# facebookresearch/esm

Hardware: NVIDIA H100
Metric: sequences/sec ESM-2 650M L=1024 embedding extract (higher is better)
Workload: dtype f16 operands, f32 accumulate/residual/LayerNorm/softmax

## Files before the change

esm_b200/csrc/attention_wg.cuh:

```cuda
#pragma once

#include "attention_common.cuh"

namespace esmb200 {

namespace attn_wg_cfg {
constexpr int BLOCK_Q = 128;
constexpr int BLOCK_KV = 128;
constexpr int STAGES = 4;
constexpr int Q_BUFS = 2;
constexpr int TILE_BYTES = 128 * 128;
constexpr int NUM_THREADS = 384;
constexpr int SMEM_BYTES = (Q_BUFS + 2 * STAGES) * TILE_BYTES + 1024 + 256;
}

__global__ void __launch_bounds__(attn_wg_cfg::NUM_THREADS, 1)
attention_wg_kernel(const __grid_constant__ CUtensorMap tmap_q, const __grid_constant__ CUtensorMap tmap_kv,
                    const AttnParams p) {
  using namespace attn_wg_cfg;
  constexpr float LOG2E = attn_cfg::LOG2E;
  constexpr int D = attn_cfg::HEAD_DIM;
  extern __shared__ uint8_t smem_raw[];
  uint8_t* smem = reinterpret_cast<uint8_t*>((reinterpret_cast<uintptr_t>(smem_raw) + 1023) & ~uintptr_t(1023));
  uint8_t* smem_q = smem;
  uint8_t* smem_k = smem + Q_BUFS * TILE_BYTES;
  uint8_t* smem_v = smem_k + STAGES * TILE_BYTES;
  uint64_t* bars = reinterpret_cast<uint64_t*>(smem_v + STAGES * TILE_BYTES);
  uint64_t* q_full = bars;
  uint64_t* q_empty = bars + Q_BUFS;
  uint64_t* k_full = bars + 2 * Q_BUFS;
  uint64_t* v_full = k_full + STAGES;
  uint64_t* kv_empty = v_full + STAGES;

  const uint32_t wg = __shfl_sync(0xffffffffu, threadIdx.x / 128, 0);
  const int nqt = (p.T + BLOCK_Q - 1) / BLOCK_Q;
  const int items = p.B * p.H * nqt;

  if (threadIdx.x == 0) {
    tma_prefetch_desc(&tmap_q);
    tma_prefetch_desc(&tmap_kv);
    for (int i = 0; i < Q_BUFS; ++i) {
      mbar_init(&q_full[i], 1);
      mbar_init(&q_empty[i], 2);
    }
    for (int i = 0; i < STAGES; ++i) {
      mbar_init(&k_full[i], 1);
      mbar_init(&v_full[i], 1);
      mbar_init(&kv_empty[i], 2);
    }
    fence_barrier_init();
  }
  __syncthreads();
  pdl_launch_dependents();
  pdl_wait();

  if (wg == 0) {
    setmaxnreg_dec<24>();
    if (threadIdx.x == 0) {
      auto wait_empty = [](uint64_t* bar, uint32_t parity) {
#if ESMB200_WATCHDOG
        uint32_t polls = 0;
        while (!mbar_try_wait(bar, parity)) {
          __nanosleep(64);
          if (++polls == (1u << 24)) __trap();
        }
#else
        while (!mbar_try_wait(bar, parity)) __nanosleep(64);
#endif
      };
      uint32_t qi = 0, it = 0;
      for (int w = blockIdx.x; w < items; w += gridDim.x) {
        const int qt = w % nqt, h = (w / nqt) % p.H, b = w / (nqt * p.H);
        const int nblk = (__ldg(p.kvlen + b) + BLOCK_KV - 1) / BLOCK_KV;
        if (nblk == 0) continue;
        const int row_base = (b / p.cols) * p.T;
        const int x0 = (b % p.cols) * 3 * p.E + h * D;
        const uint32_t qb = qi % Q_BUFS;
        wait_empty(&q_empty[qb], ((qi / Q_BUFS) & 1) ^ 1);
        mbar_arrive_expect_tx(&q_full[qb], TILE_BYTES);
        tma_load_2d(smem_q + qb * TILE_BYTES, &tmap_q, &q_full[qb], x0, row_base + qt * BLOCK_Q);
        ++qi;
        for (int j = 0; j < nblk; ++j, ++it) {
          const uint32_t s = it % STAGES;
          wait_empty(&kv_empty[s], ((it / STAGES) & 1) ^ 1);
          mbar_arrive_expect_tx(&k_full[s], TILE_BYTES);
          tma_load_2d(smem_k + s * TILE_BYTES, &tmap_kv, &k_full[s], x0 + p.E, row_base + j * BLOCK_KV);
          mbar_arrive_expect_tx(&v_full[s], TILE_BYTES);
          tma_load_2d(smem_v + s * TILE_BYTES, &tmap_kv, &v_full[s], x0 + 2 * p.E, row_base + j * BLOCK_KV);
        }
      }
    }
    return;
  }

  setmaxnreg_inc<240>();
  const uint32_t mw = wg - 1;
  const uint32_t warp = (threadIdx.x / 32) % 4;
  const uint32_t lane = threadIdx.x % 32, g = lane / 4, c = lane % 4;
  const bool signal = (threadIdx.x % 128) == 0;
  const uint32_t q_base = smem_u32(smem_q) + mw * 64 * 128;
  const uint32_t k_base = smem_u32(smem_k), v_base = smem_u32(smem_v);
  uint32_t qi = 0, it = 0;

  auto turn_begin = [&]() { named_bar_sync(1 + mw, 256); };
  auto turn_end = [&]() { named_bar_arrive(2 - mw, 256); };
  if (mw == 1) turn_end();

  auto wait_full = [](uint64_t* bar, uint32_t parity) {
#if ESMB200_WATCHDOG
    uint32_t polls = 0;
    while (!mbar_try_wait(bar, parity))
      if (++polls == (1u << 26)) __trap();
#else
    while (!mbar_try_wait(bar, parity)) {
    }
#endif
  };

  for (int w = blockIdx.x; w < items; w += gridDim.x) {
    const int qt = w % nqt, h = (w / nqt) % p.H, b = w / (nqt * p.H);
    const int nblk = (__ldg(p.kvlen + b) + BLOCK_KV - 1) / BLOCK_KV;
    const uint32_t* kb_ptr = p.keybits + (size_t)b * p.words;
    float o[32];
#pragma unroll
    for (int i = 0; i < 32; ++i) o[i] = 0.f;
    float m[2] = {-INFINITY, -INFINITY}, l[2] = {0.f, 0.f};

    if (nblk > 0) {
      const uint32_t qb = qi % Q_BUFS;
      const uint64_t dq = wgmma_desc_sw128(q_base + qb * TILE_BYTES);
      float sc[64];
      uint32_t pa[32];
      float alpha[2];

      auto issue_qk = [&](uint32_t s) {
        const uint64_t dk = wgmma_desc_sw128(k_base + s * TILE_BYTES);
        wgmma_fence();
#pragma unroll
        for (int k = 0; k < D / 16; ++k) wgmma_m64n128k16(sc, dq + 2 * k, dk + 2 * k, k);
        wgmma_commit();
      };
      auto issue_pv = [&](uint32_t s) {
#pragma unroll
        for (int i = 0; i < 8; ++i) {
          o[4 * i] *= alpha[0]; o[4 * i + 1] *= alpha[0];
          o[4 * i + 2] *= alpha[1]; o[4 * i + 3] *= alpha[1];
        }
        wgmma_fence();
        const uint64_t dv = wgmma_desc_sw128_mn(v_base + s * TILE_BYTES);
#pragma unroll
        for (int kk = 0; kk < BLOCK_KV / 16; ++kk) {
          const uint32_t a[4] = {pa[4 * kk], pa[4 * kk + 1], pa[4 * kk + 2], pa[4 * kk + 3]};
          wgmma_m64n64k16_rs(o, a, dv + kk * (2048 >> 4));
        }
        wgmma_commit();
      };
      auto softmax = [&](int j) {
        const uint4 kw = __ldg(reinterpret_cast<const uint4*>(kb_ptr + 4 * j));
        if ((kw.x & kw.y & kw.z & kw.w) != 0xffffffffu) {
          const uint32_t wd[4] = {kw.x, kw.y, kw.z, kw.w};
#pragma unroll
          for (int i = 0; i < 16; ++i)
#pragma unroll
            for (int e = 0; e < 2; ++e)
              if (!((wd[i / 4] >> ((i % 4) * 8 + 2 * c + e)) & 1u)) sc[4 * i + e] = sc[4 * i + 2 + e] = -INFINITY;
        }
        float mx[2][8];
#pragma unroll
        for (int i = 0; i < 8; ++i)
#pragma unroll
          for (int r = 0; r < 2; ++r)
            mx[r][i] = fmaxf(fmaxf(sc[4 * i + 2 * r], sc[4 * i + 2 * r + 1]),
                             fmaxf(sc[4 * (i + 8) + 2 * r], sc[4 * (i + 8) + 2 * r + 1]));
#pragma unroll
        for (int w = 4; w >= 1; w /= 2)
#pragma unroll
          for (int i = 0; i < w; ++i) {
            mx[0][i] = fmaxf(mx[0][i], mx[0][i + w]);
            mx[1][i] = fmaxf(mx[1][i], mx[1][i + w]);
          }
        float ref[2];
#pragma unroll
        for (int r = 0; r < 2; ++r) {
          const float mn = fmaxf(m[r], quad_max(mx[r][0]));
          alpha[r] = (mn == -INFINITY) ? 1.f : ex2_approx((m[r] - mn) * LOG2E);
          m[r] = mn;
          ref[r] = (mn == -INFINITY) ? 0.f : -mn * LOG2E;
          l[r] *= alpha[r];
        }
        float ls[2][4] = {{0.f, 0.f, 0.f, 0.f}, {0.f, 0.f, 0.f, 0.f}};
#pragma unroll
        for (int i = 0; i < 16; ++i)
#pragma unroll
          for (int r = 0; r < 2; ++r) {
            sc[4 * i + 2 * r] = ex2_approx(fmaf(sc[4 * i + 2 * r], LOG2E, ref[r]));
            sc[4 * i + 2 * r + 1] = ex2_approx(fmaf(sc[4 * i + 2 * r + 1], LOG2E, ref[r]));
            ls[r][i % 4] += sc[4 * i + 2 * r] + sc[4 * i + 2 * r + 1];
          }
#pragma unroll
        for (int r = 0; r < 2; ++r) l[r] += (ls[r][0] + ls[r][1]) + (ls[r][2] + ls[r][3]);
      };
      auto convert_p = [&]() {
#pragma unroll
        for (int i = 0; i < 16; ++i)
#pragma unroll
          for (int r = 0; r < 2; ++r) pa[2 * i + r] = pack_half2(sc[4 * i + 2 * r], sc[4 * i + 2 * r + 1]);
      };

      wait_full(&q_full[qb], (qi / Q_BUFS) & 1);
      ++qi;
      uint32_t s = it % STAGES;
      wait_full(&k_full[s], (it / STAGES) & 1);
      turn_begin();
      issue_qk(s);
      turn_end();
      wgmma_wait<0>();
      reg_fence_f(sc);
      if (nblk == 1 && signal) mbar_arrive(&q_empty[qb]);
      softmax(0);
      convert_p();
      wait_full(&v_full[s], (it / STAGES) & 1);
      for (int j = 1; j < nblk; ++j) {
        const uint32_t sp = s;
        ++it;
        s = it % STAGES;
        wait_full(&k_full[s], (it / STAGES) & 1);
        turn_begin();
        issue_qk(s);
        issue_pv(sp);
        turn_end();
        wgmma_wait<1>();
        reg_fence_f(sc);
        if (j == nblk - 1 && signal) mbar_arrive(&q_empty[qb]);
        softmax(j);
        wait_full(&v_full[s], (it / STAGES) & 1);
        wgmma_wait<0>();
        reg_fence_f(o);
        reg_fence_f(sc);
        if (signal) mbar_arrive(&kv_empty[sp]);
        convert_p();
      }
      turn_begin();
      issue_pv(s);
      turn_end();
      wgmma_wait<0>();
      reg_fence_f(o);
      if (signal) mbar_arrive(&kv_empty[s]);
      ++it;
    }

    const int row_base = (b / p.cols) * p.T;
#pragma unroll
    for (int r = 0; r < 2; ++r) {
      const float lr = quad_sum(l[r]);
      const int t = qt * BLOCK_Q + (int)(mw * 64 + warp * 16 + g + 8 * r);
      if (t >= p.T) continue;
      const float inv = lr > 0.f ? 1.0f / lr : 0.f;
      if (p.row_max != nullptr && c == 0) {
        const size_t si = ((size_t)b * p.H + h) * p.T + t;
        p.row_max[si] = m[r] == -INFINITY ? 0.f : m[r];
        p.row_sum[si] = lr;
      }
      __half* dst = p.ctx + ((size_t)(row_base + t) * p.cols + b % p.cols) * p.E + h * D;
#pragma unroll
      for (int i = 0; i < 8; ++i)
        *reinterpret_cast<__half2*>(dst + i * 8 + 2 * (int)c) =
            __floats2half2_rn(o[4 * i + 2 * r] * inv, o[4 * i + 2 * r + 1] * inv);
    }
  }
  if (mw == 0) turn_begin();
}

inline cudaError_t launch_attention_wg(const CUtensorMap& tmap_q, const CUtensorMap& tmap_kv, const AttnParams& p,
                                       int num_sms, cudaStream_t stream) {
  using namespace attn_wg_cfg;
  cudaError_t e = cudaFuncSetAttribute(attention_wg_kernel, cudaFuncAttributeMaxDynamicSharedMemorySize, SMEM_BYTES);
  if (e != cudaSuccess) return e;
  const long long items = (long long)p.B * p.H * ((p.T + BLOCK_Q - 1) / BLOCK_Q);
  if (items > 0x7fffffffLL) return cudaErrorInvalidConfiguration;
  const int grid = items < num_sms ? (int)items : num_sms;
  return launch_pdl(attention_wg_kernel, dim3(grid), dim3(NUM_THREADS), SMEM_BYTES, stream, tmap_q, tmap_kv, p);
}

}
```

Measured before the change: 320.1.

## Overlap final PV of previous tile with next tile's first QK in attention

```diff
diff --git a/esm_b200/csrc/attention_wg.cuh b/esm_b200/csrc/attention_wg.cuh
--- a/esm_b200/csrc/attention_wg.cuh
+++ b/esm_b200/csrc/attention_wg.cuh
@@ -117,148 +117,100 @@
 #endif
   };
 
-  for (int w = blockIdx.x; w < items; w += gridDim.x) {
+  float o[32];
+  float sc[64];
+  uint32_t pa[32];
+  float alpha[2];
+  float m[2] = {-INFINITY, -INFINITY}, l[2] = {0.f, 0.f};
+  float mp[2], lp[2];
+  uint64_t dq = 0;
+  const uint32_t* kb_ptr = p.keybits;
+
+  auto issue_qk = [&](uint32_t s) {
+    const uint64_t dk = wgmma_desc_sw128(k_base + s * TILE_BYTES);
+    wgmma_fence();
+#pragma unroll
+    for (int k = 0; k < D / 16; ++k) wgmma_m64n128k16(sc, dq + 2 * k, dk + 2 * k, k);
+    wgmma_commit();
+  };
+  auto issue_pv = [&](uint32_t s) {
+#pragma unroll
+    for (int i = 0; i < 8; ++i) {
+      o[4 * i] *= alpha[0]; o[4 * i + 1] *= alpha[0];
+      o[4 * i + 2] *= alpha[1]; o[4 * i + 3] *= alpha[1];
+    }
+    wgmma_fence();
+    const uint64_t dv = wgmma_desc_sw128_mn(v_base + s * TILE_BYTES);
+#pragma unroll
+    for (int kk = 0; kk < BLOCK_KV / 16; ++kk) {
+      const uint32_t a[4] = {pa[4 * kk], pa[4 * kk + 1], pa[4 * kk + 2], pa[4 * kk + 3]};
+      wgmma_m64n64k16_rs(o, a, dv + kk * (2048 >> 4));
+    }
+    wgmma_commit();
+  };
+  auto softmax = [&](int j) {
+    const uint4 kw = __ldg(reinterpret_cast<const uint4*>(kb_ptr + 4 * j));
+    if ((kw.x & kw.y & kw.z & kw.w) != 0xffffffffu) {
+      const uint32_t wd[4] = {kw.x, kw.y, kw.z, kw.w};
+#pragma unroll
+      for (int i = 0; i < 16; ++i)
+#pragma unroll
+        for (int e = 0; e < 2; ++e)
+          if (!((wd[i / 4] >> ((i % 4) * 8 + 2 * c + e)) & 1u)) sc[4 * i + e] = sc[4 * i + 2 + e] = -INFINITY;
+    }
+    float mx[2][8];
+#pragma unroll
+    for (int i = 0; i < 8; ++i)
+#pragma unroll
+      for (int r = 0; r < 2; ++r)
+        mx[r][i] = fmaxf(fmaxf(sc[4 * i + 2 * r], sc[4 * i + 2 * r + 1]),
+                         fmaxf(sc[4 * (i + 8) + 2 * r], sc[4 * (i + 8) + 2 * r + 1]));
+#pragma unroll
+    for (int w = 4; w >= 1; w /= 2)
+#pragma unroll
+      for (int i = 0; i < w; ++i) {
+        mx[0][i] = fmaxf(mx[0][i], mx[0][i + w]);
+        mx[1][i] = fmaxf(mx[1][i], mx[1][i + w]);
+      }
+    float ref[2];
+#pragma unroll
+    for (int r = 0; r < 2; ++r) {
+      const float mn = fmaxf(m[r], quad_max(mx[r][0]));
+      alpha[r] = (mn == -INFINITY) ? 1.f : ex2_approx((m[r] - mn) * LOG2E);
+      m[r] = mn;
+      ref[r] = (mn == -INFINITY) ? 0.f : -mn * LOG2E;
+      l[r] *= alpha[r];
+    }
+    float ls[2][4] = {{0.f, 0.f, 0.f, 0.f}, {0.f, 0.f, 0.f, 0.f}};
+#pragma unroll
+    for (int i = 0; i < 16; ++i)
+#pragma unroll
+      for (int r = 0; r < 2; ++r) {
+        sc[4 * i + 2 * r] = ex2_approx(fmaf(sc[4 * i + 2 * r], LOG2E, ref[r]));
+        sc[4 * i + 2 * r + 1] = ex2_approx(fmaf(sc[4 * i + 2 * r + 1], LOG2E, ref[r]));
+        ls[r][i % 4] += sc[4 * i + 2 * r] + sc[4 * i + 2 * r + 1];
+      }
+#pragma unroll
+    for (int r = 0; r < 2; ++r) l[r] += (ls[r][0] + ls[r][1]) + (ls[r][2] + ls[r][3]);
+  };
+  auto convert_p = [&]() {
+#pragma unroll
+    for (int i = 0; i < 16; ++i)
+#pragma unroll
+      for (int r = 0; r < 2; ++r) pa[2 * i + r] = pack_half2(sc[4 * i + 2 * r], sc[4 * i + 2 * r + 1]);
+  };
+  auto store = [&](int w, const float (&ls_)[2], const float (&ms_)[2]) {
     const int qt = w % nqt, h = (w / nqt) % p.H, b = w / (nqt * p.H);
-    const int nblk = (__ldg(p.kvlen + b) + BLOCK_KV - 1) / BLOCK_KV;
-    const uint32_t* kb_ptr = p.keybits + (size_t)b * p.words;
-    float o[32];
-#pragma unroll
-    for (int i = 0; i < 32; ++i) o[i] = 0.f;
-    float m[2] = {-INFINITY, -INFINITY}, l[2] = {0.f, 0.f};
-
-    if (nblk > 0) {
-      const uint32_t qb = qi % Q_BUFS;
-      const uint64_t dq = wgmma_desc_sw128(q_base + qb * TILE_BYTES);
-      float sc[64];
-      uint32_t pa[32];
-      float alpha[2];
-
-      auto issue_qk = [&](uint32_t s) {
-        const uint64_t dk = wgmma_desc_sw128(k_base + s * TILE_BYTES);
-        wgmma_fence();
-#pragma unroll
-        for (int k = 0; k < D / 16; ++k) wgmma_m64n128k16(sc, dq + 2 * k, dk + 2 * k, k);
-        wgmma_commit();
-      };
-      auto issue_pv = [&](uint32_t s) {
-#pragma unroll
-        for (int i = 0; i < 8; ++i) {
-          o[4 * i] *= alpha[0]; o[4 * i + 1] *= alpha[0];
-          o[4 * i + 2] *= alpha[1]; o[4 * i + 3] *= alpha[1];
-        }
-        wgmma_fence();
-        const uint64_t dv = wgmma_desc_sw128_mn(v_base + s * TILE_BYTES);
-#pragma unroll
-        for (int kk = 0; kk < BLOCK_KV / 16; ++kk) {
-          const uint32_t a[4] = {pa[4 * kk], pa[4 * kk + 1], pa[4 * kk + 2], pa[4 * kk + 3]};
-          wgmma_m64n64k16_rs(o, a, dv + kk * (2048 >> 4));
-        }
-        wgmma_commit();
-      };
-      auto softmax = [&](int j) {
-        const uint4 kw = __ldg(reinterpret_cast<const uint4*>(kb_ptr + 4 * j));
-        if ((kw.x & kw.y & kw.z & kw.w) != 0xffffffffu) {
-          const uint32_t wd[4] = {kw.x, kw.y, kw.z, kw.w};
-#pragma unroll
-          for (int i = 0; i < 16; ++i)
-#pragma unroll
-            for (int e = 0; e < 2; ++e)
-              if (!((wd[i / 4] >> ((i % 4) * 8 + 2 * c + e)) & 1u)) sc[4 * i + e] = sc[4 * i + 2 + e] = -INFINITY;
-        }
-        float mx[2][8];
-#pragma unroll
-        for (int i = 0; i < 8; ++i)
-#pragma unroll
-          for (int r = 0; r < 2; ++r)
-            mx[r][i] = fmaxf(fmaxf(sc[4 * i + 2 * r], sc[4 * i + 2 * r + 1]),
-                             fmaxf(sc[4 * (i + 8) + 2 * r], sc[4 * (i + 8) + 2 * r + 1]));
-#pragma unroll
-        for (int w = 4; w >= 1; w /= 2)
-#pragma unroll
-          for (int i = 0; i < w; ++i) {
-            mx[0][i] = fmaxf(mx[0][i], mx[0][i + w]);
-            mx[1][i] = fmaxf(mx[1][i], mx[1][i + w]);
-          }
-        float ref[2];
-#pragma unroll
-        for (int r = 0; r < 2; ++r) {
-          const float mn = fmaxf(m[r], quad_max(mx[r][0]));
-          alpha[r] = (mn == -INFINITY) ? 1.f : ex2_approx((m[r] - mn) * LOG2E);
-          m[r] = mn;
-          ref[r] = (mn == -INFINITY) ? 0.f : -mn * LOG2E;
-          l[r] *= alpha[r];
-        }
-        float ls[2][4] = {{0.f, 0.f, 0.f, 0.f}, {0.f, 0.f, 0.f, 0.f}};
-#pragma unroll
-        for (int i = 0; i < 16; ++i)
-#pragma unroll
-          for (int r = 0; r < 2; ++r) {
-            sc[4 * i + 2 * r] = ex2_approx(fmaf(sc[4 * i + 2 * r], LOG2E, ref[r]));
-            sc[4 * i + 2 * r + 1] = ex2_approx(fmaf(sc[4 * i + 2 * r + 1], LOG2E, ref[r]));
-            ls[r][i % 4] += sc[4 * i + 2 * r] + sc[4 * i + 2 * r + 1];
-          }
-#pragma unroll
-        for (int r = 0; r < 2; ++r) l[r] += (ls[r][0] + ls[r][1]) + (ls[r][2] + ls[r][3]);
-      };
-      auto convert_p = [&]() {
-#pragma unroll
-        for (int i = 0; i < 16; ++i)
-#pragma unroll
-          for (int r = 0; r < 2; ++r) pa[2 * i + r] = pack_half2(sc[4 * i + 2 * r], sc[4 * i + 2 * r + 1]);
-      };
-
-      wait_full(&q_full[qb], (qi / Q_BUFS) & 1);
-      ++qi;
-      uint32_t s = it % STAGES;
-      wait_full(&k_full[s], (it / STAGES) & 1);
-      turn_begin();
-      issue_qk(s);
-      turn_end();
-      wgmma_wait<0>();
-      reg_fence_f(sc);
-      if (nblk == 1 && signal) mbar_arrive(&q_empty[qb]);
-      softmax(0);
-      convert_p();
-      wait_full(&v_full[s], (it / STAGES) & 1);
-      for (int j = 1; j < nblk; ++j) {
-        const uint32_t sp = s;
-        ++it;
-        s = it % STAGES;
-        wait_full(&k_full[s], (it / STAGES) & 1);
-        turn_begin();
-        issue_qk(s);
-        issue_pv(sp);
-        turn_end();
-        wgmma_wait<1>();
-        reg_fence_f(sc);
-        if (j == nblk - 1 && signal) mbar_arrive(&q_empty[qb]);
-        softmax(j);
-        wait_full(&v_full[s], (it / STAGES) & 1);
-        wgmma_wait<0>();
-        reg_fence_f(o);
-        reg_fence_f(sc);
-        if (signal) mbar_arrive(&kv_empty[sp]);
-        convert_p();
-      }
-      turn_begin();
-      issue_pv(s);
-      turn_end();
-      wgmma_wait<0>();
-      reg_fence_f(o);
-      if (signal) mbar_arrive(&kv_empty[s]);
-      ++it;
-    }
-
     const int row_base = (b / p.cols) * p.T;
 #pragma unroll
     for (int r = 0; r < 2; ++r) {
-      const float lr = quad_sum(l[r]);
+      const float lr = quad_sum(ls_[r]);
       const int t = qt * BLOCK_Q + (int)(mw * 64 + warp * 16 + g + 8 * r);
       if (t >= p.T) continue;
       const float inv = lr > 0.f ? 1.0f / lr : 0.f;
       if (p.row_max != nullptr && c == 0) {
         const size_t si = ((size_t)b * p.H + h) * p.T + t;
-        p.row_max[si] = m[r] == -INFINITY ? 0.f : m[r];
+        p.row_max[si] = ms_[r] == -INFINITY ? 0.f : ms_[r];
         p.row_sum[si] = lr;
       }
       __half* dst = p.ctx + ((size_t)(row_base + t) * p.cols + b % p.cols) * p.E + h * D;
@@ -267,6 +219,100 @@
         *reinterpret_cast<__half2*>(dst + i * 8 + 2 * (int)c) =
             __floats2half2_rn(o[4 * i + 2 * r] * inv, o[4 * i + 2 * r + 1] * inv);
     }
+  };
+
+  int pw = -1;
+  uint32_t ps = 0;
+#pragma unroll
+  for (int i = 0; i < 32; ++i) {
+    o[i] = 0.f;
+    pa[i] = 0u;
+  }
+  alpha[0] = alpha[1] = 0.f;
+  for (int w = blockIdx.x; w < items; w += gridDim.x) {
+    const int b = w / (nqt * p.H), h = (w / nqt) % p.H, t0 = (w % nqt) * BLOCK_Q;
+    if (__ldg(p.kvlen + b) > 0) continue;
+    const int rows = min(BLOCK_Q, p.T - t0), r0 = (int)(mw * 64 + warp * 16 + g);
+    for (int r = r0; r < min(rows, r0 + 9); r += 8) {
+      const int t = t0 + r;
+      if (p.row_max != nullptr && c == 0) {
+        const size_t si = ((size_t)b * p.H + h) * p.T + t;
+        p.row_max[si] = p.row_sum[si] = 0.f;
+      }
+      __half* dst = p.ctx + ((size_t)((b / p.cols) * p.T + t) * p.cols + b % p.cols) * p.E + h * D + 16 * (int)c;
+      reinterpret_cast<uint4*>(dst)[0] = make_uint4(0u, 0u, 0u, 0u);
+      reinterpret_cast<uint4*>(dst)[1] = make_uint4(0u, 0u, 0u, 0u);
+    }
+  }
+  for (int w = blockIdx.x; w < items; w += gridDim.x) {
+    const int b = w / (nqt * p.H);
+    const int nblk = (__ldg(p.kvlen + b) + BLOCK_KV - 1) / BLOCK_KV;
+    if (nblk == 0) continue;
+    kb_ptr = p.keybits + (size_t)b * p.words;
+    const uint32_t qb = qi % Q_BUFS;
+    dq = wgmma_desc_sw128(q_base + qb * TILE_BYTES);
+    wait_full(&q_full[qb], (qi / Q_BUFS) & 1);
+    ++qi;
+    uint32_t s = it % STAGES;
+    wait_full(&k_full[s], (it / STAGES) & 1);
+    turn_begin();
+    issue_qk(s);
+    issue_pv(ps);
+    turn_end();
+    wgmma_wait<1>();
+    reg_fence_f(sc);
+    if (nblk == 1 && signal) mbar_arrive(&q_empty[qb]);
+#pragma unroll
+    for (int r = 0; r < 2; ++r) {
+      lp[r] = l[r];
+      mp[r] = m[r];
+      m[r] = -INFINITY;
+      l[r] = 0.f;
+    }
+    softmax(0);
+    wait_full(&v_full[s], (it / STAGES) & 1);
+    wgmma_wait<0>();
+    reg_fence_f(o);
+    if (pw >= 0) {
+      if (signal) mbar_arrive(&kv_empty[ps]);
+      store(pw, lp, mp);
+    }
+#pragma unroll
+    for (int i = 0; i < 32; ++i) o[i] = 0.f;
+    reg_fence_f(sc);
+    convert_p();
+    for (int j = 1; j < nblk; ++j) {
+      const uint32_t sp = s;
+      ++it;
+      s = it % STAGES;
+      wait_full(&k_full[s], (it / STAGES) & 1);
+      turn_begin();
+      issue_qk(s);
+      issue_pv(sp);
+      turn_end();
+      wgmma_wait<1>();
+      reg_fence_f(sc);
+      if (j == nblk - 1 && signal) mbar_arrive(&q_empty[qb]);
+      softmax(j);
+      wait_full(&v_full[s], (it / STAGES) & 1);
+      wgmma_wait<0>();
+      reg_fence_f(o);
+      reg_fence_f(sc);
+      if (signal) mbar_arrive(&kv_empty[sp]);
+      convert_p();
+    }
+    ++it;
+    pw = w;
+    ps = s;
+  }
+  turn_begin();
+  issue_pv(ps);
+  turn_end();
+  wgmma_wait<0>();
+  reg_fence_f(o);
+  if (pw >= 0) {
+    if (signal) mbar_arrive(&kv_empty[ps]);
+    store(pw, l, m);
   }
   if (mw == 0) turn_begin();
 }
```

New measurement: 321.0 (median of 6 runs). About the same (+0.3%).
